# A-Nasiri-M/sap3d_tensorflow

Hardware: AMD Instinct MI355X
Metric: clips/s (16x112x112 fwd+bwd) (higher is better)
Workload: dtype f32

## Files before the change

### sap3d_tensorflow_amd/csrc/elementwise.hip

```cpp
#include "p3d_kernels.h"
#include "det_reduce.h"
#define P3D_SEED(a) ((a).seed_dev ? *(a).seed_dev : (a).seed)

namespace {

__device__ __forceinline__ float4 ld4(const float* p) { return *reinterpret_cast<const float4*>(p); }
__device__ __forceinline__ void st4(float* p, float4 v) { *reinterpret_cast<float4*>(p) = v; }
__device__ __forceinline__ float4 f4(float a) { return make_float4(a, a, a, a); }
__device__ __forceinline__ float4 fma4(float4 a, float4 b, float4 c) {
    return make_float4(fmaf(a.x, b.x, c.x), fmaf(a.y, b.y, c.y), fmaf(a.z, b.z, c.z), fmaf(a.w, b.w, c.w));
}
__device__ __forceinline__ float4 add4(float4 a, float4 b) { return make_float4(a.x + b.x, a.y + b.y, a.z + b.z, a.w + b.w); }
__device__ __forceinline__ float4 sub4(float4 a, float4 b) { return make_float4(a.x - b.x, a.y - b.y, a.z - b.z, a.w - b.w); }
__device__ __forceinline__ float4 mul4(float4 a, float4 b) { return make_float4(a.x * b.x, a.y * b.y, a.z * b.z, a.w * b.w); }
__device__ __forceinline__ float4 relu4(float4 a) { return make_float4(fmaxf(a.x, 0.f), fmaxf(a.y, 0.f), fmaxf(a.z, 0.f), fmaxf(a.w, 0.f)); }
__device__ __forceinline__ float4 gate4(float4 g, float4 pre) {
    return make_float4(pre.x > 0.f ? g.x : 0.f, pre.y > 0.f ? g.y : 0.f, pre.z > 0.f ? g.z : 0.f, pre.w > 0.f ? g.w : 0.f);
}

__device__ __forceinline__ float u01(unsigned long long seed, unsigned long long idx) {
    unsigned long long z = seed + 0x9E3779B97F4A7C15ull * (idx + 1);
    z = (z ^ (z >> 30)) * 0xBF58476D1CE4E5B9ull;
    z = (z ^ (z >> 27)) * 0x94D049BB133111EBull;
    z ^= z >> 31;
    return (float)(z >> 40) * (1.0f / 16777216.0f);
}
__device__ __forceinline__ float4 dropmask4(unsigned long long seed, long long e0, float rate, float scale) {
    return make_float4(u01(seed, e0) >= rate ? scale : 0.f, u01(seed, e0 + 1) >= rate ? scale : 0.f,
                       u01(seed, e0 + 2) >= rate ? scale : 0.f, u01(seed, e0 + 3) >= rate ? scale : 0.f);
}

static_assert(P3D_STAT_REPLICAS == 16, "finalize kernels fold 16 replicas with 4 shuffle steps");
__device__ __forceinline__ double fold16(double v) {
#pragma unroll
    for (int o = 8; o > 0; o >>= 1) v += __shfl_xor(v, o);
    return v;
}
template <int LPC>
__global__ __launch_bounds__(256) void bn_finalize_kernel(BnParams bn, double invM, int use_batch, int update_moving, float eps) {
    P3D_CHAIN_PRIO();
    const int r = threadIdx.x % LPC;
    const int c = blockIdx.x * (256 / LPC) + threadIdx.x / LPC;
    const bool ok = c < bn.C;
    double s1 = 0.0, s2 = 0.0;
    if (use_batch) {
        if (ok) {
            const float2* part = reinterpret_cast<const float2*>(bn.statpart) + c;
#pragma unroll 4
            for (int q = r; q < bn.nparts; q += LPC) {
                const float2 v = part[(size_t)q * bn.C];
                s1 += (double)v.x; s2 += (double)v.y;
            }
        }
#pragma unroll
        for (int o = LPC / 2; o > 0; o >>= 1) { s1 += __shfl_xor(s1, o); s2 += __shfl_xor(s2, o); }
    }
    if (!ok || r) return;
    double mean, var;
    if (use_batch) {
        mean = s1 * invM;
        var = s2 * invM - mean * mean;
        if (var < 0.0) var = 0.0;
        if (update_moving) {
            bn.moving_mean[c] -= (bn.moving_mean[c] - (float)mean) * (1.0f - 0.99f);
            bn.moving_var[c] -= (bn.moving_var[c] - (float)var) * (1.0f - 0.99f);
        }
    } else {
        mean = bn.moving_mean[c];
        var = bn.moving_var[c];
    }
    const double inv = 1.0 / sqrt(var + (double)eps);
    const float sc = (float)((double)bn.gamma[c] * inv);
    bn.scale[c] = sc;
    bn.shift[c] = (float)((double)bn.beta[c] - mean * (double)bn.gamma[c] * inv);
    bn.mean[c] = (float)mean;
    bn.invstd[c] = (float)inv;
}

__global__ __launch_bounds__(256) void bn_stats_kernel(const float* y, int ld, long long M, int C, float* statpart) {
    P3D_CHAIN_PRIO();
    __shared__ float red[256][8];
    const int c4n = C >> 2;
    const int rpi = 256 / c4n;
    const int tid = threadIdx.x;
    const int sub = tid / c4n;
    const int cg = tid - sub * c4n;
    const int c = cg << 2;
    float4 s1 = f4(0.f), s2 = f4(0.f);
    if (sub < rpi)
        for (long long row = (long long)blockIdx.x * rpi + sub; row < M; row += (long long)gridDim.x * rpi) {
            const float4 v = ld4(y + row * ld + c);
            s1 = add4(s1, v);
            s2 = fma4(v, v, s2);
        }
    float* r = red[tid];
    r[0] = s1.x; r[1] = s1.y; r[2] = s1.z; r[3] = s1.w; r[4] = s2.x; r[5] = s2.y; r[6] = s2.z; r[7] = s2.w;
    __syncthreads();
    if (tid < c4n) {
        float t[8];
#pragma unroll
        for (int q = 0; q < 8; ++q) t[q] = 0.f;
        for (int s = 0; s < rpi; ++s)
#pragma unroll
            for (int q = 0; q < 8; ++q) t[q] += red[s * c4n + tid][q];
        float* st = statpart + (size_t)blockIdx.x * 2 * C;
#pragma unroll
        for (int q = 0; q < 4; ++q) { st[2 * (c + q) + 0] = t[q]; st[2 * (c + q) + 1] = t[4 + q]; }
    }
}

template <int MODE>
__global__ __launch_bounds__(256) void bn_apply_kernel(BnApplyArgs a) {
    p3d_warm_kernarg_lines<(int)(sizeof(BnApplyArgs) / 64)>();
    P3D_CHAIN_PRIO();
    const int c4n = a.C >> 2;
    const long long total = a.M * c4n;
    for (long long i = (long long)blockIdx.x * blockDim.x + threadIdx.x; i < total; i += (long long)gridDim.x * blockDim.x) {
        const long long row = i / c4n;
        const int c = (int)(i - row * c4n) << 2;
        float4 v = fma4(ld4(a.scale1 + c), ld4(a.y1 + row * a.ld1 + c), ld4(a.shift1 + c));
        float4 z;
        if (MODE == 0) z = relu4(v);
        else if (MODE == 1) z = relu4(add4(v, ld4(a.y2 + row * a.ld2 + c)));
        else if (MODE == 2) z = relu4(add4(v, fma4(ld4(a.scale2 + c), ld4(a.y2 + row * a.ld2 + c), ld4(a.shift2 + c))));
        else if (MODE == 3) z = add4(relu4(v), relu4(fma4(ld4(a.scale2 + c), ld4(a.y2 + row * a.ld2 + c), ld4(a.shift2 + c))));
        else z = add4(ld4(a.y2 + row * a.ld2 + c), relu4(v));
        if (a.drop_scale > 0.f) z = mul4(z, dropmask4(P3D_SEED(a), row * a.C + c, a.drop_rate, a.drop_scale));
        st4(a.z + row * a.ldz + c, z);
    }
}

__device__ __forceinline__ void bn_fold64(const BnParams& bn, int c0, double invM, int use_batch, int update_moving, float eps, bool publish,
                                          float* sc_lds, float* sh_lds) {
    const int ch = c0 + (threadIdx.x >> 2), r = threadIdx.x & 3;
    double s1 = 0.0, s2 = 0.0;
    if (use_batch) {
        const float2* part = reinterpret_cast<const float2*>(bn.statpart) + ch;
#pragma unroll 8
        for (int q = r; q < bn.nparts; q += 4) {
            const float2 v = part[(size_t)q * bn.C];
            s1 += (double)v.x; s2 += (double)v.y;
        }
        s1 += __shfl_xor(s1, 1); s2 += __shfl_xor(s2, 1);
        s1 += __shfl_xor(s1, 2); s2 += __shfl_xor(s2, 2);
    }
    if (r) return;
    double mean, var;
    if (use_batch) {
        mean = s1 * invM;
        var = s2 * invM - mean * mean;
        if (var < 0.0) var = 0.0;
        if (publish && update_moving) {
            bn.moving_mean[ch] -= (bn.moving_mean[ch] - (float)mean) * (1.0f - 0.99f);
            bn.moving_var[ch] -= (bn.moving_var[ch] - (float)var) * (1.0f - 0.99f);
        }
    } else {
        mean = bn.moving_mean[ch];
        var = bn.moving_var[ch];
    }
    const double inv = 1.0 / sqrt(var + (double)eps);
    const float sc = (float)((double)bn.gamma[ch] * inv);
    const float sh = (float)((double)bn.beta[ch] - mean * (double)bn.gamma[ch] * inv);
    sc_lds[ch - c0] = sc; sh_lds[ch - c0] = sh;
    if (publish) { bn.scale[ch] = sc; bn.shift[ch] = sh; bn.mean[ch] = (float)mean; bn.invstd[ch] = (float)inv; }
}

template <int MODE>
__global__ __launch_bounds__(256) void bn_fold_apply_kernel(BnApplyArgs a, BnParams bn1, BnParams bn2, double invM, int batch1, int batch2,
                                                           int update_moving, float eps, int rows_per_block) {
    p3d_warm_kernarg_lines<(int)((sizeof(BnApplyArgs) + 2 * sizeof(BnParams)) / 64)>();
    P3D_CHAIN_PRIO();
    constexpr bool TWO = (MODE == 2 || MODE == 3);
    __shared__ __attribute__((aligned(16))) float sc1[64], sh1[64], sc2[64], sh2[64];
    const int c0 = blockIdx.y * 64;
    const bool publish = blockIdx.x == 0;
    bn_fold64(bn1, c0, invM, batch1, update_moving, eps, publish, sc1, sh1);
    if (TWO) bn_fold64(bn2, c0, invM, batch2, update_moving, eps, publish, sc2, sh2);
    __syncthreads();
    const int cl = (threadIdx.x & 15) << 2, c = c0 + cl;
    const float4 s1v = ld4(sc1 + cl), h1v = ld4(sh1 + cl);
    float4 s2v = f4(0.f), h2v = f4(0.f);
    if (TWO) { s2v = ld4(sc2 + cl); h2v = ld4(sh2 + cl); }
    const long long r0 = (long long)blockIdx.x * rows_per_block;
    const long long r1 = r0 + rows_per_block < a.M ? r0 + rows_per_block : a.M;
    for (long long row = r0 + (threadIdx.x >> 4); row < r1; row += 16) {
        const float4 v = fma4(s1v, ld4(a.y1 + row * a.ld1 + c), h1v);
        float4 z;
        if (MODE == 0) z = relu4(v);
        else if (MODE == 1) z = relu4(add4(v, ld4(a.y2 + row * a.ld2 + c)));
        else if (MODE == 2) z = relu4(add4(v, fma4(s2v, ld4(a.y2 + row * a.ld2 + c), h2v)));
        else if (MODE == 3) z = add4(relu4(v), relu4(fma4(s2v, ld4(a.y2 + row * a.ld2 + c), h2v)));
        else z = add4(ld4(a.y2 + row * a.ld2 + c), relu4(v));
        st4(a.z + row * a.ldz + c, z);
    }
}

template <int MODE>
__device__ __forceinline__ void bn_bwd_gates(const BnBwdArgs& a, long long row, int c, float4& g1, float4& g2,
                                             float4& y1, float4& y2) {
    float4 dz = ld4(a.dz + row * a.lddz + c);
    if (a.drop_scale > 0.f) dz = mul4(dz, dropmask4(P3D_SEED(a), row * a.C + c, a.drop_rate, a.drop_scale));
    y1 = ld4(a.y1 + row * a.ld1 + c);
    const float4 v1 = fma4(ld4(a.scale1 + c), y1, ld4(a.shift1 + c));
    y2 = f4(0.f);
    if (MODE == 0) { g1 = gate4(dz, v1); g2 = f4(0.f); }
    else if (MODE == 1) { y2 = ld4(a.y2 + row * a.ld2 + c); g1 = gate4(dz, add4(v1, y2)); g2 = g1; }
    else if (MODE == 2) {
        y2 = ld4(a.y2 + row * a.ld2 + c);
        const float4 v2 = fma4(ld4(a.scale2 + c), y2, ld4(a.shift2 + c));
        g1 = gate4(dz, add4(v1, v2)); g2 = g1;
    } else if (MODE == 3) {
        y2 = ld4(a.y2 + row * a.ld2 + c);
        const float4 v2 = fma4(ld4(a.scale2 + c), y2, ld4(a.shift2 + c));
        g1 = gate4(dz, v1); g2 = gate4(dz, v2);
    } else { g1 = gate4(dz, v1); g2 = dz; }
}

template <int MODE>
__global__ __launch_bounds__(256) void bn_bwd_reduce_kernel(BnBwdArgs a) {
    p3d_warm_kernarg_lines<(int)(sizeof(BnBwdArgs) / 64)>();
    P3D_CHAIN_PRIO();
    constexpr bool TWO = (MODE == 2 || MODE == 3);
    __shared__ float red[256][TWO ? 16 : 8];
    const int c4n = a.C >> 2;
    const int rpi = 256 / c4n;
    const int tid = threadIdx.x;
    const int sub = tid / c4n;
    const int cg = tid - sub * c4n;
    const int c = cg << 2;
    const bool active = sub < rpi;
    float4 s1 = f4(0.f), sx1 = f4(0.f), s2 = f4(0.f), sx2 = f4(0.f);
    if (active) {
        const float4 m1 = ld4(a.mean1 + c), i1 = ld4(a.invstd1 + c);
        float4 m2 = f4(0.f), i2 = f4(0.f);
        if (TWO) { m2 = ld4(a.mean2 + c); i2 = ld4(a.invstd2 + c); }
        const long long stride = (long long)gridDim.x * rpi;
        float4 t1 = f4(0.f), tx1 = f4(0.f), t2 = f4(0.f), tx2 = f4(0.f);
        long long row = (long long)blockIdx.x * rpi + sub;
        for (; row + stride < a.M; row += 2 * stride) {
            float4 g1, g2, y1, y2, h1, h2, z1, z2;
            bn_bwd_gates<MODE>(a, row, c, g1, g2, y1, y2);
            bn_bwd_gates<MODE>(a, row + stride, c, h1, h2, z1, z2);
            s1 = add4(s1, g1);
            sx1 = fma4(g1, mul4(sub4(y1, m1), i1), sx1);
            t1 = add4(t1, h1);
            tx1 = fma4(h1, mul4(sub4(z1, m1), i1), tx1);
            if (TWO) {
                s2 = add4(s2, g2);
                sx2 = fma4(g2, mul4(sub4(y2, m2), i2), sx2);
                t2 = add4(t2, h2);
                tx2 = fma4(h2, mul4(sub4(z2, m2), i2), tx2);
            }
        }
        if (row < a.M) {
            float4 g1, g2, y1, y2;
            bn_bwd_gates<MODE>(a, row, c, g1, g2, y1, y2);
            s1 = add4(s1, g1);
            sx1 = fma4(g1, mul4(sub4(y1, m1), i1), sx1);
            if (TWO) {
                s2 = add4(s2, g2);
                sx2 = fma4(g2, mul4(sub4(y2, m2), i2), sx2);
            }
        }
        s1 = add4(s1, t1); sx1 = add4(sx1, tx1);
        if (TWO) { s2 = add4(s2, t2); sx2 = add4(sx2, tx2); }
    }
    float* r = red[tid];
    r[0] = s1.x; r[1] = s1.y; r[2] = s1.z; r[3] = s1.w; r[4] = sx1.x; r[5] = sx1.y; r[6] = sx1.z; r[7] = sx1.w;
    if (TWO) { r[8] = s2.x; r[9] = s2.y; r[10] = s2.z; r[11] = s2.w; r[12] = sx2.x; r[13] = sx2.y; r[14] = sx2.z; r[15] = sx2.w; }
    __syncthreads();
    if (tid < c4n) {
        constexpr int NV = TWO ? 16 : 8;
        float t[NV];
#pragma unroll
        for (int q = 0; q < NV; ++q) t[q] = 0.f;
        for (int s = 0; s < rpi; ++s)
#pragma unroll
            for (int q = 0; q < NV; ++q) t[q] += red[s * c4n + tid][q];
        float* p1 = a.part1 + ((size_t)blockIdx.x * a.C + c) * 2;
#pragma unroll
        for (int q = 0; q < 4; ++q) { p1[2 * q] = t[q]; p1[2 * q + 1] = t[4 + q]; }
        if (TWO) {
            float* p2 = a.part2 + ((size_t)blockIdx.x * a.C + c) * 2;
#pragma unroll
            for (int q = 0; q < 4; ++q) { p2[2 * q] = t[8 + q]; p2[2 * q + 1] = t[12 + q]; }
        }
    }
}

template <int LPC>
__global__ __launch_bounds__(256) void bn_bwd_finalize_kernel(BnBwdArgs a, int two) {
    p3d_warm_kernarg_lines<(int)(sizeof(BnBwdArgs) / 64)>();
    P3D_CHAIN_PRIO();
    const int r = threadIdx.x % LPC;
    const int c = blockIdx.x * (256 / LPC) + threadIdx.x / LPC;
    const bool ok = c < a.C;
    const double invM = 1.0 / (double)a.M;
    double s1 = 0.0, s2 = 0.0, t1 = 0.0, t2 = 0.0;
    if (ok) {
        const float2* p1 = reinterpret_cast<const float2*>(a.part1) + c;
        const float2* p2 = reinterpret_cast<const float2*>(a.part2) + c;
#pragma unroll 4
        for (int q = r; q < a.nparts; q += LPC) {
            const float2 v = p1[(size_t)q * a.C];
            s1 += (double)v.x; s2 += (double)v.y;
            if (two) { const float2 w = p2[(size_t)q * a.C]; t1 += (double)w.x; t2 += (double)w.y; }
        }
    }
#pragma unroll
    for (int o = LPC / 2; o > 0; o >>= 1) {
        s1 += __shfl_xor(s1, o); s2 += __shfl_xor(s2, o);
        if (two) { t1 += __shfl_xor(t1, o); t2 += __shfl_xor(t2, o); }
    }
    if (!ok || r) return;
    a.dbeta1[c] = (float)s1; a.dgamma1[c] = (float)s2;
    a.coef1[2 * c] = (float)(s1 * invM); a.coef1[2 * c + 1] = (float)(s2 * invM);
    if (two) {
        a.dbeta2[c] = (float)t1; a.dgamma2[c] = (float)t2;
        a.coef2[2 * c] = (float)(t1 * invM); a.coef2[2 * c + 1] = (float)(t2 * invM);
    }
}

__global__ __launch_bounds__(256) void bn_grad_finalize_kernel(BnGradFold f) {
    P3D_CHAIN_PRIO();
    const int r = threadIdx.x & 15;
    const int c = blockIdx.x * 16 + (threadIdx.x >> 4);
    const bool ok = c < f.C;
    double sg = 0.0, sgx = 0.0;
    if (ok) {
        const float2* part = reinterpret_cast<const float2*>(f.part) + c;
#pragma unroll 4
        for (int q = r; q < f.nparts; q += 16) {
            const float2 v = part[(size_t)q * f.C];
            sg += (double)v.x; sgx += (double)v.y;
        }
    }
    sg = fold16(sg); sgx = fold16(sgx);
    if (!ok || r) return;
    const float inv = f.invstd[c];
    const float c1 = (float)(sg * f.inv_m), c2 = (float)(sgx * f.inv_m);
    const float k1 = f.gamma[c] * inv;
    const float k2 = -k1 * inv * c2;
    const float k3 = -k1 * c1 - k2 * f.mean[c];
    f.coef[c] = k1; f.coef[f.C + c] = k2; f.coef[2 * f.C + c] = k3;
    f.dgamma[c] = (float)sgx; f.dbeta[c] = (float)sg;
}

__device__ __forceinline__ void ldcoef(const float* coef, int c, float4& c1, float4& c2) {
    const float4 lo = ld4(coef + 2 * c), hi = ld4(coef + 2 * c + 4);
    c1 = make_float4(lo.x, lo.z, hi.x, hi.z);
    c2 = make_float4(lo.y, lo.w, hi.y, hi.w);
}

template <int MODE>
__global__ __launch_bounds__(256) void bn_bwd_apply_kernel(BnBwdArgs a) {
    p3d_warm_kernarg_lines<(int)(sizeof(BnBwdArgs) / 64)>();
    P3D_CHAIN_PRIO();
    constexpr bool TWO = (MODE == 2 || MODE == 3);
    const int c4n = a.C >> 2;
    const long long total = a.M * c4n;
    const long long gtid = (long long)blockIdx.x * blockDim.x + threadIdx.x;
    for (long long i = gtid; i < total; i += (long long)gridDim.x * blockDim.x) {
        const long long row = i / c4n;
        const int c = (int)(i - row * c4n) << 2;
        float4 g1, g2, y1, y2;
        bn_bwd_gates<MODE>(a, row, c, g1, g2, y1, y2);
        {
            const float4 k = mul4(ld4(a.gamma1 + c), ld4(a.invstd1 + c));
            float4 d;
            if (a.batch1) {
                const float4 xh = mul4(sub4(y1, ld4(a.mean1 + c)), ld4(a.invstd1 + c));
                float4 c1, c2;
                ldcoef(a.coef1, c, c1, c2);
                d = mul4(k, sub4(sub4(g1, c1), mul4(xh, c2)));
            } else d = mul4(k, g1);
            float* dst = a.dy1 + row * a.lddy1 + c;
            if (a.acc1) d = add4(d, ld4(dst));
            st4(dst, d);
        }
        if (MODE != 0) {
            float4 d;
            if (TWO) {
                const float4 k = mul4(ld4(a.gamma2 + c), ld4(a.invstd2 + c));
                if (a.batch2) {
                    const float4 xh = mul4(sub4(y2, ld4(a.mean2 + c)), ld4(a.invstd2 + c));
                    float4 c1, c2;
                    ldcoef(a.coef2, c, c1, c2);
                    d = mul4(k, sub4(sub4(g2, c1), mul4(xh, c2)));
                } else d = mul4(k, g2);
            } else d = g2;
            float* dst = a.dy2 + row * a.lddy2 + c;
            if (a.acc2) d = add4(d, ld4(dst));
            st4(dst, d);
        }
    }
}

__global__ __launch_bounds__(256) void maxpool_fwd_kernel(PoolArgs a) {
    p3d_warm_kernarg_lines<(int)(sizeof(PoolArgs) / 64)>();
    P3D_CHAIN_PRIO();
    const int c4n = a.C >> 2;
    const long long total = (long long)a.N * a.Do * a.Ho * a.Wo * c4n;
    for (long long i = (long long)blockIdx.x * blockDim.x + threadIdx.x; i < total; i += (long long)gridDim.x * blockDim.x) {
        long long pos = i / c4n;
        const int c = (int)(i - pos * c4n) << 2;
        const long long opos = pos;
        const int ow = (int)(pos % a.Wo); pos /= a.Wo;
        const int oh = (int)(pos % a.Ho); pos /= a.Ho;
        const int od = (int)(pos % a.Do); const int n = (int)(pos / a.Do);
        float4 best = f4(-INFINITY);
        unsigned bx = 0, by = 0, bz = 0, bw = 0;
        for (int kd = 0; kd < a.kd; ++kd) {
            const int id = od * a.sd - a.pd + kd;
            if ((unsigned)id >= (unsigned)a.Di) continue;
            for (int kh = 0; kh < a.kh; ++kh) {
                const int ih = oh * a.sh - a.ph + kh;
                if ((unsigned)ih >= (unsigned)a.Hi) continue;
                for (int kw = 0; kw < a.kw; ++kw) {
                    const int iw = ow * a.sw - a.pw + kw;
                    if ((unsigned)iw >= (unsigned)a.Wi) continue;
                    const float4 v = ld4(a.x + ((((long long)n * a.Di + id) * a.Hi + ih) * a.Wi + iw) * a.ldx + c);
                    const unsigned t = (unsigned)((kd * a.kh + kh) * a.kw + kw);
                    if (v.x > best.x) { best.x = v.x; bx = t; }
                    if (v.y > best.y) { best.y = v.y; by = t; }
                    if (v.z > best.z) { best.z = v.z; bz = t; }
                    if (v.w > best.w) { best.w = v.w; bw = t; }
                }
            }
        }
        st4(a.y + opos * a.ldy + c, best);
        if (a.idx) a.idx[opos * c4n + (c >> 2)] = bx | (by << 8) | (bz << 16) | (bw << 24);
    }
}

template <int KIND>
__device__ __forceinline__ float loss_term(float z, float p, float t, int through_sigmoid, float& g) {
    if (KIND == 1) {
        g = (through_sigmoid ? p : 1.f / (1.f + expf(-z))) - t;
        return fmaxf(z, 0.f) - z * t + log1pf(expf(-fabsf(z)));
    }
    const float d = p - t;
    const float ad = fabsf(d);
    const bool quad = KIND == 0 && ad < 1.f;
    g = quad ? d : (d > 0.f ? 1.f : (d < 0.f ? -1.f : 0.f));
    if (through_sigmoid) g *= p * (1.f - p);
    return KIND == 2 ? ad : (quad ? 0.5f * d * d : ad - 0.5f);
}

template <int KIND>
__device__ __forceinline__ void loss_body(const float* logits, const float* pred, const float* target, long long n,
                                          double* loss_out, float* dl, int through_sigmoid, int vec4, double* part,
                                          unsigned* counter) {
    __shared__ double wsum[4];
    __shared__ int last_flag;
    double acc = 0.0;
    const bool need_z = KIND == 1, need_p = KIND != 1 || through_sigmoid;
    const long long gtid = (long long)blockIdx.x * blockDim.x + threadIdx.x, gsz = (long long)gridDim.x * blockDim.x;
    if (vec4) {
        const long long n4 = n >> 2;
        for (long long i = gtid; i < n4; i += gsz) {
            const float4 z = need_z ? ld4(logits + 4 * i) : f4(0.f), p = need_p ? ld4(pred + 4 * i) : f4(0.f);
            const float4 t = ld4(target + 4 * i);
            float4 g;
            acc += loss_term<KIND>(z.x, p.x, t.x, through_sigmoid, g.x);
            acc += loss_term<KIND>(z.y, p.y, t.y, through_sigmoid, g.y);
            acc += loss_term<KIND>(z.z, p.z, t.z, through_sigmoid, g.z);
            acc += loss_term<KIND>(z.w, p.w, t.w, through_sigmoid, g.w);
            st4(dl + 4 * i, g);
        }
    } else {
        for (long long i = gtid; i < n; i += gsz)
            acc += loss_term<KIND>(need_z ? logits[i] : 0.f, need_p ? pred[i] : 0.f, target[i], through_sigmoid, dl[i]);
    }
    const double bsum = p3d_block_sum<false>(acc, wsum);
    if (threadIdx.x == 0) p3d_store_wt(part, blockIdx.x, bsum);
    if (!p3d_last_block_wt(counter, gridDim.x, &last_flag)) return;
    double t = 0.0;
    for (unsigned b = threadIdx.x; b < gridDim.x; b += 256) t += part[b];
    t = p3d_block_sum<true>(t, wsum);
    if (threadIdx.x == 0) *loss_out += t;
}
__global__ __launch_bounds__(256) void smooth_l1_kernel(const float* pred, const float* target, long long n,
                                                        double* loss_out, float* dl, int through_sigmoid, int vec4, double* part,
                                                        unsigned* counter) {
    P3D_CHAIN_PRIO();
    loss_body<0>(nullptr, pred, target, n, loss_out, dl, through_sigmoid, vec4, part, counter);
}
__global__ __launch_bounds__(256) void sigmoid_ce_kernel(const float* logits, const float* pred, const float* target, long long n,
                                                         double* loss_out, float* dl, int through_sigmoid, int vec4, double* part,
                                                         unsigned* counter) {
    P3D_CHAIN_PRIO();
    loss_body<1>(logits, pred, target, n, loss_out, dl, through_sigmoid, vec4, part, counter);
}
__global__ __launch_bounds__(256) void l1_loss_kernel(const float* logits, const float* pred, const float* target, long long n,
                                                      double* loss_out, float* dl, int through_sigmoid, int vec4, double* part,
                                                      unsigned* counter) {
// ... 289 lines not shown
        const long long st = gridDim.x;
        for (; row + 7 * st < M; row += 8 * st) {
            float v[8];
#pragma unroll
            for (int u = 0; u < 8; ++u) v[u] = dy[(row + u * st) * ld + c];
#pragma unroll
            for (int u = 0; u < 8; ++u) acc += v[u];
        }
        for (; row < M; row += st) acc += dy[row * ld + c];
        p3d_store_wt(part, (size_t)blockIdx.x * C + c, acc);
    }
    if (!p3d_last_block_wt(counters + blockIdx.y, gridDim.x, &last_flag)) return;
    if (c >= C) return;
    float t = 0.f;
    unsigned b = 0;
    for (; b + 7 < gridDim.x; b += 8) {
        float v[8];
#pragma unroll
        for (int u = 0; u < 8; ++u) v[u] = part[(size_t)(b + u) * C + c];
#pragma unroll
        for (int u = 0; u < 8; ++u) t += v[u];
    }
    for (; b < gridDim.x; ++b) t += part[(size_t)b * C + c];
    out[c] += t;
}

__global__ __launch_bounds__(256) void colsum4_kernel(const float* __restrict__ dy, int ld, long long M, int C, float* out,
                                                      float* part, unsigned* counters) {
    __shared__ float4 red[256];
    __shared__ int last_flag;
    const int L = C >> 2, R = 256 / L;
    const int lane = threadIdx.x % L, rs = threadIdx.x / L;
    const bool live = rs < R;
    float4 acc = make_float4(0.f, 0.f, 0.f, 0.f);
    if (live) {
        const long long stride = (long long)gridDim.x * R;
        long long row = (long long)blockIdx.x * R + rs;
        const float* base = dy + lane * 4;
        for (; row + 7 * stride < M; row += 8 * stride) {
            float4 v[8];
#pragma unroll
            for (int u = 0; u < 8; ++u) v[u] = *reinterpret_cast<const float4*>(base + (row + u * stride) * ld);
#pragma unroll
            for (int u = 0; u < 8; ++u) { acc.x += v[u].x; acc.y += v[u].y; acc.z += v[u].z; acc.w += v[u].w; }
        }
        for (; row < M; row += stride) {
            const float4 v = *reinterpret_cast<const float4*>(base + row * ld);
            acc.x += v.x; acc.y += v.y; acc.z += v.z; acc.w += v.w;
        }
    }
    red[threadIdx.x] = acc;
    __syncthreads();
    if (threadIdx.x < L) {
        float4 t = red[threadIdx.x];
        for (int r = 1; r < R; ++r) { const float4 v = red[r * L + threadIdx.x]; t.x += v.x; t.y += v.y; t.z += v.z; t.w += v.w; }
        p3d_store_wt4(part, (size_t)blockIdx.x * C + threadIdx.x * 4, t);
    }
    if (!p3d_last_block_wt(counters, gridDim.x, &last_flag)) return;
    acc = make_float4(0.f, 0.f, 0.f, 0.f);
    if (live) {
        const float* src = part + lane * 4;
        unsigned b = rs;
        for (; b + 7u * R < gridDim.x; b += 8u * R) {
            float4 v[8];
#pragma unroll
            for (int u = 0; u < 8; ++u) v[u] = *reinterpret_cast<const float4*>(src + (size_t)(b + u * R) * C);
#pragma unroll
            for (int u = 0; u < 8; ++u) { acc.x += v[u].x; acc.y += v[u].y; acc.z += v[u].z; acc.w += v[u].w; }
        }
        for (; b < gridDim.x; b += R) {
            const float4 v = *reinterpret_cast<const float4*>(src + (size_t)b * C);
            acc.x += v.x; acc.y += v.y; acc.z += v.z; acc.w += v.w;
        }
    }
    __syncthreads();
    red[threadIdx.x] = acc;
    __syncthreads();
    if (threadIdx.x < L) {
        float4 t = red[threadIdx.x];
        for (int r = 1; r < R; ++r) { const float4 v = red[r * L + threadIdx.x]; t.x += v.x; t.y += v.y; t.z += v.z; t.w += v.w; }
        float4* o = reinterpret_cast<float4*>(out + threadIdx.x * 4);
        float4 cur = *o;
        cur.x += t.x; cur.y += t.y; cur.z += t.z; cur.w += t.w;
        *o = cur;
    }
}

inline unsigned grid_for(long long total, int per_block = 256, int cap = 4096) {
    long long b = (total + per_block - 1) / per_block;
    if (b < 1) b = 1;
    if (b > cap) b = cap;
    return (unsigned)b;
}

}

hipError_t p3d_bn_finalize(const BnParams& bn, long M, int use_batch, int update_moving, float eps, hipStream_t s) {
    if (use_batch && (!bn.statpart || bn.nparts < 1)) return hipErrorInvalidValue;
    if (use_batch && bn.nparts > 64)
        hipLaunchKernelGGL(bn_finalize_kernel<64>, dim3((bn.C + 3) / 4), dim3(256), 0, s, bn, 1.0 / (double)M, use_batch, update_moving, eps);
    else
        hipLaunchKernelGGL(bn_finalize_kernel<16>, dim3((bn.C + 15) / 16), dim3(256), 0, s, bn, 1.0 / (double)M, use_batch, update_moving, eps);
    return hipGetLastError();
}

int p3d_bn_stats_parts(long M, int C) {
    if ((C & 3) || C > 1024 || C < 4) return 0;
    const int rpi = 256 / (C >> 2);
    long long blocks = (M + (long long)rpi * 8 - 1) / ((long long)rpi * 8);
    if (blocks < 1) blocks = 1;
    if (blocks > 512) blocks = 512;
    return (int)blocks;
}

hipError_t p3d_bn_stats(const float* y, int ld, long M, int C, float* statpart, hipStream_t s) {
    if ((C & 3) || C > 1024 || (ld & 3)) return hipErrorInvalidValue;
    const long long blocks = p3d_bn_stats_parts(M, C);
    hipLaunchKernelGGL(bn_stats_kernel, dim3((unsigned)blocks), dim3(256), 0, s, y, ld, (long long)M, C, statpart);
    return hipGetLastError();
}

hipError_t p3d_bn_apply(const BnApplyArgs& a, hipStream_t s) {
    if ((a.C & 3) || (a.ld1 & 3) || (a.ldz & 3)) return hipErrorInvalidValue;
    const unsigned g = grid_for(a.M * (a.C >> 2));
    switch (a.mode) {
        case 0: hipLaunchKernelGGL(bn_apply_kernel<0>, dim3(g), dim3(256), 0, s, a); break;
        case 1: hipLaunchKernelGGL(bn_apply_kernel<1>, dim3(g), dim3(256), 0, s, a); break;
        case 2: hipLaunchKernelGGL(bn_apply_kernel<2>, dim3(g), dim3(256), 0, s, a); break;
        case 3: hipLaunchKernelGGL(bn_apply_kernel<3>, dim3(g), dim3(256), 0, s, a); break;
        case 4: hipLaunchKernelGGL(bn_apply_kernel<4>, dim3(g), dim3(256), 0, s, a); break;
        default: return hipErrorInvalidValue;
    }
    return hipGetLastError();
}

bool p3d_bn_fold_apply_ok(long M, int C, int nparts1, int nparts2, float drop_scale) {
    static const bool off = p3d_tune_env("P3D_BN_FOLD_APPLY") && atoi(p3d_tune_env("P3D_BN_FOLD_APPLY")) == 0;
    return !off && (C % 64) == 0 && nparts1 <= 128 && nparts2 <= 128 && M >= 1024 && !(drop_scale > 0.f);
}
hipError_t p3d_bn_fold_apply(const BnApplyArgs& a, const BnParams& bn1, const BnParams& bn2, int batch1, int batch2, int update_moving,
                             float eps, hipStream_t s) {
    const bool two = a.mode == 2 || a.mode == 3;
    if ((a.ld1 & 3) || (a.ldz & 3) || !p3d_bn_fold_apply_ok(a.M, a.C, batch1 ? bn1.nparts : 0, two && batch2 ? bn2.nparts : 0, a.drop_scale))
        return hipErrorInvalidValue;
    if ((batch1 && (!bn1.statpart || bn1.nparts < 1)) || (two && batch2 && (!bn2.statpart || bn2.nparts < 1))) return hipErrorInvalidValue;
    const int groups = a.C / 64;
    int chunks = 256 / groups;
    if (chunks < 1) chunks = 1;
    long rows = (a.M + chunks - 1) / chunks;
    rows = (rows + 15) / 16 * 16;
    chunks = (int)((a.M + rows - 1) / rows);
    const dim3 g((unsigned)chunks, (unsigned)groups);
    const double invM = 1.0 / (double)a.M;
#define P3D_FA(M_) case M_: hipLaunchKernelGGL(bn_fold_apply_kernel<M_>, g, dim3(256), 0, s, a, bn1, bn2, invM, batch1, batch2, update_moving, eps, (int)rows); break;
    switch (a.mode) { P3D_FA(0) P3D_FA(1) P3D_FA(2) P3D_FA(3) P3D_FA(4) default: return hipErrorInvalidValue; }
#undef P3D_FA
    return hipGetLastError();
}

int p3d_bn_bwd_parts(long M, int C) {
    if ((C & 3) || C > 1024 || C < 4) return 0;
    const int rpi = 256 / (C >> 2);
    long long blocks = (M + (long long)rpi * 8 - 1) / ((long long)rpi * 8);
    if (blocks < 1) blocks = 1;
    if (blocks > 512) blocks = 512;
    return (int)blocks;
}

hipError_t p3d_bn_bwd_reduce(const BnBwdArgs& a, hipStream_t s) {
    if ((a.C & 3) || a.C > 1024 || !a.part1 || a.nparts != p3d_bn_bwd_parts(a.M, a.C)) return hipErrorInvalidValue;
    const unsigned g = (unsigned)a.nparts;
    switch (a.mode) {
        case 0: hipLaunchKernelGGL(bn_bwd_reduce_kernel<0>, dim3(g), dim3(256), 0, s, a); break;
        case 1: hipLaunchKernelGGL(bn_bwd_reduce_kernel<1>, dim3(g), dim3(256), 0, s, a); break;
        case 2: hipLaunchKernelGGL(bn_bwd_reduce_kernel<2>, dim3(g), dim3(256), 0, s, a); break;
        case 3: hipLaunchKernelGGL(bn_bwd_reduce_kernel<3>, dim3(g), dim3(256), 0, s, a); break;
        case 4: hipLaunchKernelGGL(bn_bwd_reduce_kernel<4>, dim3(g), dim3(256), 0, s, a); break;
        default: return hipErrorInvalidValue;
    }
    return hipGetLastError();
}

hipError_t p3d_bn_bwd_finalize(const BnBwdArgs& a, hipStream_t s) {
    const int two = (a.mode == 2 || a.mode == 3) ? 1 : 0;
    if (a.nparts >= 64) hipLaunchKernelGGL(bn_bwd_finalize_kernel<64>, dim3((a.C + 3) / 4), dim3(256), 0, s, a, two);
    else hipLaunchKernelGGL(bn_bwd_finalize_kernel<16>, dim3((a.C + 15) / 16), dim3(256), 0, s, a, two);
    return hipGetLastError();
}

hipError_t p3d_bn_grad_finalize(const BnGradFold& f, hipStream_t s) {
    if (!f.part || f.nparts <= 0) return hipErrorInvalidValue;
    hipLaunchKernelGGL(bn_grad_finalize_kernel, dim3((f.C + 15) / 16), dim3(256), 0, s, f);
    return hipGetLastError();
}

hipError_t p3d_bn_bwd_apply(const BnBwdArgs& a, hipStream_t s) {
    if (a.C & 3) return hipErrorInvalidValue;
    unsigned g = grid_for(a.M * (a.C >> 2));
    switch (a.mode) {
        case 0: hipLaunchKernelGGL(bn_bwd_apply_kernel<0>, dim3(g), dim3(256), 0, s, a); break;
        case 1: hipLaunchKernelGGL(bn_bwd_apply_kernel<1>, dim3(g), dim3(256), 0, s, a); break;
        case 2: hipLaunchKernelGGL(bn_bwd_apply_kernel<2>, dim3(g), dim3(256), 0, s, a); break;
        case 3: hipLaunchKernelGGL(bn_bwd_apply_kernel<3>, dim3(g), dim3(256), 0, s, a); break;
        case 4: hipLaunchKernelGGL(bn_bwd_apply_kernel<4>, dim3(g), dim3(256), 0, s, a); break;
        default: return hipErrorInvalidValue;
    }
    return hipGetLastError();
}

hipError_t p3d_maxpool_fwd(const PoolArgs& a, hipStream_t s) {
    if (a.C & 3) return hipErrorInvalidValue;
    const long long total = (long long)a.N * a.Do * a.Ho * a.Wo * (a.C >> 2);
    hipLaunchKernelGGL(maxpool_fwd_kernel, dim3(grid_for(total)), dim3(256), 0, s, a);
    return hipGetLastError();
}

__global__ __launch_bounds__(256) void maxpool_bwd_disjoint_kernel(PoolArgs a, int accumulate) {
    p3d_warm_kernarg_lines<(int)(sizeof(PoolArgs) / 64)>();
    P3D_CHAIN_PRIO();
    const int c4n = a.C >> 2;
    const long long total = (long long)a.N * a.Do * a.Ho * a.Wo * c4n;
    for (long long i = (long long)blockIdx.x * blockDim.x + threadIdx.x; i < total; i += (long long)gridDim.x * blockDim.x) {
        long long pos = i / c4n;
        const int c = (int)(i - pos * c4n) << 2;
        const long long opos = pos;
        const int ow = (int)(pos % a.Wo); pos /= a.Wo;
        const int oh = (int)(pos % a.Ho); pos /= a.Ho;
        const int od = (int)(pos % a.Do); const int n = (int)(pos / a.Do);
        const float4 g = ld4(a.dy + opos * a.lddy + c);
        const float4 y = ld4(a.y + opos * a.ldy + c);
        float4 left = g;
        bool done[4] = {false, false, false, false};
        for (int kd = 0; kd < a.kd; ++kd)
            for (int kh = 0; kh < a.kh; ++kh)
                for (int kw = 0; kw < a.kw; ++kw) {
                    const long long ipos = (((long long)n * a.Di + od * a.sd + kd) * a.Hi + oh * a.sh + kh) * a.Wi + ow * a.sw + kw;
                    const float4 v = ld4(a.x + ipos * a.ldx + c);
                    float4 d = f4(0.f);
                    if (!done[0] && v.x == y.x) { d.x = left.x; done[0] = true; }
                    if (!done[1] && v.y == y.y) { d.y = left.y; done[1] = true; }
                    if (!done[2] && v.z == y.z) { d.z = left.z; done[2] = true; }
                    if (!done[3] && v.w == y.w) { d.w = left.w; done[3] = true; }
                    float* dst = a.dx + ipos * a.lddx + c;
                    if (accumulate) d = add4(d, ld4(dst));
                    st4(dst, d);
                }
    }
}

__global__ __launch_bounds__(256) void maxpool_bwd_gather_kernel(PoolArgs a, int accumulate) {
    p3d_warm_kernarg_lines<(int)(sizeof(PoolArgs) / 64)>();
    P3D_CHAIN_PRIO();
    const int c4n = a.C >> 2;
    const long long total = (long long)a.N * a.Di * a.Hi * a.Wi * c4n;
    for (long long i = (long long)blockIdx.x * blockDim.x + threadIdx.x; i < total; i += (long long)gridDim.x * blockDim.x) {
        long long pos = i / c4n;
        const int c = (int)(i - pos * c4n) << 2;
        const long long ipos = pos;
        const int iw = (int)(pos % a.Wi); pos /= a.Wi;
        const int ih = (int)(pos % a.Hi); pos /= a.Hi;
        const int id = (int)(pos % a.Di); const int n = (int)(pos / a.Di);
        const int pdv = id + a.pd, phv = ih + a.ph, pwv = iw + a.pw;
        float4 acc = f4(0.f);
        if (a.kd <= 2 * a.sd && a.kh <= 2 * a.sh && a.kw <= 2 * a.sw) {
            int od2[2], oh2[2], ow2[2];
            bool vd[2], vh[2], vw[2];
#pragma unroll
            for (int q = 0; q < 2; ++q) {
                od2[q] = pdv / a.sd - q; vd[q] = od2[q] >= 0 && od2[q] < a.Do && pdv - od2[q] * a.sd < a.kd;
                oh2[q] = phv / a.sh - q; vh[q] = oh2[q] >= 0 && oh2[q] < a.Ho && phv - oh2[q] * a.sh < a.kh;
                ow2[q] = pwv / a.sw - q; vw[q] = ow2[q] >= 0 && ow2[q] < a.Wo && pwv - ow2[q] * a.sw < a.kw;
            }
            unsigned wd[8]; float4 g8[8]; unsigned t8[8]; bool ok[8];
#pragma unroll
            for (int q = 0; q < 8; ++q) {
                const int qd = q >> 2, qh = (q >> 1) & 1, qw = q & 1;
                ok[q] = vd[qd] && vh[qh] && vw[qw];
                t8[q] = (unsigned)(((pdv - od2[qd] * a.sd) * a.kh + (phv - oh2[qh] * a.sh)) * a.kw + (pwv - ow2[qw] * a.sw));
                const long long opos = ok[q] ? (((long long)n * a.Do + od2[qd]) * a.Ho + oh2[qh]) * a.Wo + ow2[qw] : 0;
                wd[q] = ok[q] ? a.idx[opos * c4n + (c >> 2)] : 0xffffffffu;
                g8[q] = ok[q] ? ld4(a.dy + opos * a.lddy + c) : f4(0.f);
            }
#pragma unroll
            for (int q = 0; q < 8; ++q) {
                if (!ok[q]) continue;
                const unsigned w = wd[q], t = t8[q];
                if ((w & 255u) == t) acc.x += g8[q].x;
                if (((w >> 8) & 255u) == t) acc.y += g8[q].y;
                if (((w >> 16) & 255u) == t) acc.z += g8[q].z;
                if ((w >> 24) == t) acc.w += g8[q].w;
            }
        } else
        for (int od = pdv / a.sd; od >= 0 && pdv - od * a.sd < a.kd; --od) {
            if (od >= a.Do) continue;
            for (int oh = phv / a.sh; oh >= 0 && phv - oh * a.sh < a.kh; --oh) {
                if (oh >= a.Ho) continue;
                for (int ow = pwv / a.sw; ow >= 0 && pwv - ow * a.sw < a.kw; --ow) {
                    if (ow >= a.Wo) continue;
                    const unsigned t = (unsigned)(((pdv - od * a.sd) * a.kh + (phv - oh * a.sh)) * a.kw + (pwv - ow * a.sw));
                    const long long opos = (((long long)n * a.Do + od) * a.Ho + oh) * a.Wo + ow;
                    const unsigned w = a.idx[opos * c4n + (c >> 2)];
                    const float4 g = ld4(a.dy + opos * a.lddy + c);
                    if ((w & 255u) == t) acc.x += g.x;
                    if (((w >> 8) & 255u) == t) acc.y += g.y;
                    if (((w >> 16) & 255u) == t) acc.z += g.z;
                    if ((w >> 24) == t) acc.w += g.w;
                }
            }
        }
        float* dst = a.dx + ipos * a.lddx + c;
        if (accumulate) acc = add4(acc, ld4(dst));
        st4(dst, acc);
    }
}

bool p3d_maxpool_disjoint(const PoolArgs& a) {
    return a.kd == a.sd && a.kh == a.sh && a.kw == a.sw && a.pd == 0 && a.ph == 0 && a.pw == 0 &&
           a.Do * a.sd == a.Di && a.Ho * a.sh == a.Hi && a.Wo * a.sw == a.Wi;
}

hipError_t p3d_maxpool_bwd_disjoint(const PoolArgs& a, int accumulate, hipStream_t s) {
    if ((a.C & 3) || !p3d_maxpool_disjoint(a)) return hipErrorInvalidValue;
    const long long total = (long long)a.N * a.Do * a.Ho * a.Wo * (a.C >> 2);
    hipLaunchKernelGGL(maxpool_bwd_disjoint_kernel, dim3(grid_for(total)), dim3(256), 0, s, a, accumulate);
    return hipGetLastError();
}


static uintptr_t low4(const void* q) { return reinterpret_cast<uintptr_t>(q) & 15; }

LaunchDesc p3d_loss_desc(const LossArgs& a) {
    const double n = (double)a.n;
// ... 245 lines not shown
```

Baseline: 536.2.

## Batch-issue partial-stat and activation loads ahead of reductions in BN kernels

Introduces a PartLoads helper that issues all partial-sum loads up front, with clamped indices, before accumulating them in double. It is used in the BN finalize, backward finalize, grad finalize and fold-apply kernels, and gamma/beta/moving stats are also loaded early. The fold-apply kernel now prefetches several activation rows before finishing the stat fold, so global latency overlaps the fold. The backward reduce adds a single-pass prefetch variant for modes 0 and 4 when each thread covers at most 8 rows. The cost is more registers and more template instantiations, with occupancy risk for the larger prefetch depths.

```diff
diff --git a/sap3d_tensorflow_amd/csrc/elementwise.hip b/sap3d_tensorflow_amd/csrc/elementwise.hip
--- a/sap3d_tensorflow_amd/csrc/elementwise.hip
+++ b/sap3d_tensorflow_amd/csrc/elementwise.hip
@@ -36,43 +36,75 @@
     for (int o = 8; o > 0; o >>= 1) v += __shfl_xor(v, o);
     return v;
 }
+template <int N, int LPC, int TN = N>
+struct PartLoads {
+    float2 v[N];
+    __device__ __forceinline__ void issue(const float2* part, int nparts, int C, int r) {
+#pragma unroll
+        for (int j = 0; j < N; ++j) v[j] = part[(size_t)min(r + j * LPC, nparts - 1) * C];
+    }
+    __device__ __forceinline__ void add(const float2* part, int nparts, int C, int r, double& s1, double& s2) {
+        __builtin_amdgcn_sched_barrier(0);
+#pragma unroll
+        for (int j = 0; j < N; ++j) asm volatile("" : "+v"(v[j].x), "+v"(v[j].y) : : "memory");
+#pragma unroll
+        for (int j = 0; j < N; ++j)
+            if (r + j * LPC < nparts) { s1 += (double)v[j].x; s2 += (double)v[j].y; }
+        for (int q = r + N * LPC; q < nparts; q += TN * LPC) {
+            float2 w[TN];
+#pragma unroll
+            for (int j = 0; j < TN; ++j) w[j] = part[(size_t)min(q + j * LPC, nparts - 1) * C];
+#pragma unroll
+            for (int j = 0; j < TN; ++j)
+                if (q + j * LPC < nparts) { s1 += (double)w[j].x; s2 += (double)w[j].y; }
+        }
+    }
+};
+
 template <int LPC>
 __global__ __launch_bounds__(256) void bn_finalize_kernel(BnParams bn, double invM, int use_batch, int update_moving, float eps) {
+    p3d_warm_kernarg_lines<(int)((sizeof(BnParams) + sizeof(double) + 2 * sizeof(int) + sizeof(float) + 63) / 64)>();
     P3D_CHAIN_PRIO();
+    constexpr int N = LPC == 64 ? 8 : 4;
+    constexpr int TN = LPC == 64 ? 16 : 4;
     const int r = threadIdx.x % LPC;
     const int c = blockIdx.x * (256 / LPC) + threadIdx.x / LPC;
     const bool ok = c < bn.C;
+    const bool last = ok && r == 0;
+    float g = 0.f, b = 0.f, mm = 0.f, mv = 0.f;
+    if (last) {
+        g = bn.gamma[c]; b = bn.beta[c];
+        if (!use_batch || update_moving) { mm = bn.moving_mean[c]; mv = bn.moving_var[c]; }
+    }
     double s1 = 0.0, s2 = 0.0;
     if (use_batch) {
         if (ok) {
             const float2* part = reinterpret_cast<const float2*>(bn.statpart) + c;
-#pragma unroll 4
-            for (int q = r; q < bn.nparts; q += LPC) {
-                const float2 v = part[(size_t)q * bn.C];
-                s1 += (double)v.x; s2 += (double)v.y;
-            }
+            PartLoads<N, LPC, TN> p;
+            p.issue(part, bn.nparts, bn.C, r);
+            p.add(part, bn.nparts, bn.C, r, s1, s2);
         }
 #pragma unroll
         for (int o = LPC / 2; o > 0; o >>= 1) { s1 += __shfl_xor(s1, o); s2 += __shfl_xor(s2, o); }
     }
-    if (!ok || r) return;
+    if (!last) return;
     double mean, var;
     if (use_batch) {
         mean = s1 * invM;
         var = s2 * invM - mean * mean;
         if (var < 0.0) var = 0.0;
         if (update_moving) {
-            bn.moving_mean[c] -= (bn.moving_mean[c] - (float)mean) * (1.0f - 0.99f);
-            bn.moving_var[c] -= (bn.moving_var[c] - (float)var) * (1.0f - 0.99f);
+            bn.moving_mean[c] = mm - (mm - (float)mean) * (1.0f - 0.99f);
+            bn.moving_var[c] = mv - (mv - (float)var) * (1.0f - 0.99f);
         }
     } else {
-        mean = bn.moving_mean[c];
-        var = bn.moving_var[c];
+        mean = mm;
+        var = mv;
     }
     const double inv = 1.0 / sqrt(var + (double)eps);
-    const float sc = (float)((double)bn.gamma[c] * inv);
+    const float sc = (float)((double)g * inv);
     bn.scale[c] = sc;
-    bn.shift[c] = (float)((double)bn.beta[c] - mean * (double)bn.gamma[c] * inv);
+    bn.shift[c] = (float)((double)b - mean * (double)g * inv);
     bn.mean[c] = (float)mean;
     bn.invstd[c] = (float)inv;
 }
@@ -130,17 +162,25 @@
     }
 }
 
-__device__ __forceinline__ void bn_fold64(const BnParams& bn, int c0, double invM, int use_batch, int update_moving, float eps, bool publish,
-                                          float* sc_lds, float* sh_lds) {
+struct BnFold64 {
+    PartLoads<32, 4> p;
+    float g, b, mm, mv;
+};
+__device__ __forceinline__ void bn_fold64_issue(BnFold64& f, const BnParams& bn, int c0, int use_batch, int update_moving, bool publish) {
+    const int ch = c0 + (threadIdx.x >> 2), r = threadIdx.x & 3;
+    f.g = f.b = f.mm = f.mv = 0.f;
+    if (use_batch) f.p.issue(reinterpret_cast<const float2*>(bn.statpart) + ch, bn.nparts, bn.C, r);
+    if (r == 0) {
+        f.g = bn.gamma[ch]; f.b = bn.beta[ch];
+        if (!use_batch || (publish && update_moving)) { f.mm = bn.moving_mean[ch]; f.mv = bn.moving_var[ch]; }
+    }
+}
+__device__ __forceinline__ void bn_fold64_finish(BnFold64& f, const BnParams& bn, int c0, double invM, int use_batch, int update_moving,
+                                                 float eps, bool publish, float* sc_lds, float* sh_lds) {
     const int ch = c0 + (threadIdx.x >> 2), r = threadIdx.x & 3;
     double s1 = 0.0, s2 = 0.0;
     if (use_batch) {
-        const float2* part = reinterpret_cast<const float2*>(bn.statpart) + ch;
-#pragma unroll 8
-        for (int q = r; q < bn.nparts; q += 4) {
-            const float2 v = part[(size_t)q * bn.C];
-            s1 += (double)v.x; s2 += (double)v.y;
-        }
+        f.p.add(reinterpret_cast<const float2*>(bn.statpart) + ch, bn.nparts, bn.C, r, s1, s2);
         s1 += __shfl_xor(s1, 1); s2 += __shfl_xor(s2, 1);
         s1 += __shfl_xor(s1, 2); s2 += __shfl_xor(s2, 2);
     }
@@ -151,47 +191,70 @@
         var = s2 * invM - mean * mean;
         if (var < 0.0) var = 0.0;
         if (publish && update_moving) {
-            bn.moving_mean[ch] -= (bn.moving_mean[ch] - (float)mean) * (1.0f - 0.99f);
-            bn.moving_var[ch] -= (bn.moving_var[ch] - (float)var) * (1.0f - 0.99f);
+            bn.moving_mean[ch] = f.mm - (f.mm - (float)mean) * (1.0f - 0.99f);
+            bn.moving_var[ch] = f.mv - (f.mv - (float)var) * (1.0f - 0.99f);
         }
     } else {
-        mean = bn.moving_mean[ch];
-        var = bn.moving_var[ch];
+        mean = f.mm;
+        var = f.mv;
     }
     const double inv = 1.0 / sqrt(var + (double)eps);
-    const float sc = (float)((double)bn.gamma[ch] * inv);
-    const float sh = (float)((double)bn.beta[ch] - mean * (double)bn.gamma[ch] * inv);
+    const float sc = (float)((double)f.g * inv);
+    const float sh = (float)((double)f.b - mean * (double)f.g * inv);
     sc_lds[ch - c0] = sc; sh_lds[ch - c0] = sh;
     if (publish) { bn.scale[ch] = sc; bn.shift[ch] = sh; bn.mean[ch] = (float)mean; bn.invstd[ch] = (float)inv; }
 }
 
 template <int MODE>
+__device__ __forceinline__ float4 bn_fold_apply_row(float4 y1, float4 y2, float4 s1v, float4 h1v, float4 s2v, float4 h2v) {
+    const float4 v = fma4(s1v, y1, h1v);
+    if (MODE == 0) return relu4(v);
+    else if (MODE == 1) return relu4(add4(v, y2));
+    else if (MODE == 2) return relu4(add4(v, fma4(s2v, y2, h2v)));
+    else if (MODE == 3) return add4(relu4(v), relu4(fma4(s2v, y2, h2v)));
+    else return add4(y2, relu4(v));
+}
+
+template <int MODE, int PF>
 __global__ __launch_bounds__(256) void bn_fold_apply_kernel(BnApplyArgs a, BnParams bn1, BnParams bn2, double invM, int batch1, int batch2,
                                                            int update_moving, float eps, int rows_per_block) {
     p3d_warm_kernarg_lines<(int)((sizeof(BnApplyArgs) + 2 * sizeof(BnParams)) / 64)>();
     P3D_CHAIN_PRIO();
     constexpr bool TWO = (MODE == 2 || MODE == 3);
+    constexpr int NPF = PF > 0 ? PF : 1;
     __shared__ __attribute__((aligned(16))) float sc1[64], sh1[64], sc2[64], sh2[64];
+    if (PF > 0) batch1 = batch2 = 1;
     const int c0 = blockIdx.y * 64;
     const bool publish = blockIdx.x == 0;
-    bn_fold64(bn1, c0, invM, batch1, update_moving, eps, publish, sc1, sh1);
-    if (TWO) bn_fold64(bn2, c0, invM, batch2, update_moving, eps, publish, sc2, sh2);
+    const int cl = (threadIdx.x & 15) << 2, c = c0 + cl;
+    const long long r0 = (long long)blockIdx.x * rows_per_block;
+    const long long r1 = r0 + rows_per_block < a.M ? r0 + rows_per_block : a.M;
+    const long long row0 = r0 + (threadIdx.x >> 4);
+    BnFold64 f1, f2;
+    bn_fold64_issue(f1, bn1, c0, batch1, update_moving, publish);
+    if (TWO) bn_fold64_issue(f2, bn2, c0, batch2, update_moving, publish);
+    float4 y1v[NPF], y2v[NPF];
+#pragma unroll
+    for (int j = 0; j < PF; ++j) {
+        const long long row = row0 + 16 * j < a.M ? row0 + 16 * j : a.M - 1;
+        y1v[j] = ld4(a.y1 + row * a.ld1 + c);
+        y2v[j] = MODE != 0 ? ld4(a.y2 + row * a.ld2 + c) : f4(0.f);
+    }
+    bn_fold64_finish(f1, bn1, c0, invM, batch1, update_moving, eps, publish, sc1, sh1);
+    if (TWO) bn_fold64_finish(f2, bn2, c0, invM, batch2, update_moving, eps, publish, sc2, sh2);
     __syncthreads();
-    const int cl = (threadIdx.x & 15) << 2, c = c0 + cl;
     const float4 s1v = ld4(sc1 + cl), h1v = ld4(sh1 + cl);
     float4 s2v = f4(0.f), h2v = f4(0.f);
     if (TWO) { s2v = ld4(sc2 + cl); h2v = ld4(sh2 + cl); }
-    const long long r0 = (long long)blockIdx.x * rows_per_block;
-    const long long r1 = r0 + rows_per_block < a.M ? r0 + rows_per_block : a.M;
-    for (long long row = r0 + (threadIdx.x >> 4); row < r1; row += 16) {
-        const float4 v = fma4(s1v, ld4(a.y1 + row * a.ld1 + c), h1v);
-        float4 z;
-        if (MODE == 0) z = relu4(v);
-        else if (MODE == 1) z = relu4(add4(v, ld4(a.y2 + row * a.ld2 + c)));
-        else if (MODE == 2) z = relu4(add4(v, fma4(s2v, ld4(a.y2 + row * a.ld2 + c), h2v)));
-        else if (MODE == 3) z = add4(relu4(v), relu4(fma4(s2v, ld4(a.y2 + row * a.ld2 + c), h2v)));
-        else z = add4(ld4(a.y2 + row * a.ld2 + c), relu4(v));
-        st4(a.z + row * a.ldz + c, z);
+#pragma unroll
+    for (int j = 0; j < PF; ++j) {
+        const long long row = row0 + 16 * j;
+        if (row < r1) st4(a.z + row * a.ldz + c, bn_fold_apply_row<MODE>(y1v[j], y2v[j], s1v, h1v, s2v, h2v));
+    }
+    for (long long row = row0 + 16 * PF; row < r1; row += 16) {
+        float4 y2 = f4(0.f);
+        if (MODE != 0) y2 = ld4(a.y2 + row * a.ld2 + c);
+        st4(a.z + row * a.ldz + c, bn_fold_apply_row<MODE>(ld4(a.y1 + row * a.ld1 + c), y2, s1v, h1v, s2v, h2v));
     }
 }
 
@@ -216,7 +279,7 @@
     } else { g1 = gate4(dz, v1); g2 = dz; }
 }
 
-template <int MODE>
+template <int MODE, bool PRE>
 __global__ __launch_bounds__(256) void bn_bwd_reduce_kernel(BnBwdArgs a) {
     p3d_warm_kernarg_lines<(int)(sizeof(BnBwdArgs) / 64)>();
     P3D_CHAIN_PRIO();
@@ -237,7 +300,31 @@
         const long long stride = (long long)gridDim.x * rpi;
         float4 t1 = f4(0.f), tx1 = f4(0.f), t2 = f4(0.f), tx2 = f4(0.f);
         long long row = (long long)blockIdx.x * rpi + sub;
-        for (; row + stride < a.M; row += 2 * stride) {
+        if constexpr (PRE) {
+            static_assert(MODE == 0 || MODE == 4, "the sums of modes 1-3 read y2 as well: the loop");
+            const float4 sc1 = ld4(a.scale1 + c), sh1 = ld4(a.shift1 + c);
+            const unsigned long long seed = a.drop_scale > 0.f ? P3D_SEED(a) : 0ull;
+            float4 dzv[8], y1v[8];
+#pragma unroll
+            for (int k = 0; k < 8; ++k) {
+                const long long rk = row + k * stride < a.M ? row + k * stride : a.M - 1;
+                dzv[k] = ld4(a.dz + rk * a.lddz + c);
+                y1v[k] = ld4(a.y1 + rk * a.ld1 + c);
+            }
+#pragma unroll
+            for (int k = 0; k < 8; ++k) {
+                const long long rk = row + k * stride;
+                if (rk < a.M) {
+                    float4 dz = dzv[k];
+                    if (a.drop_scale > 0.f) dz = mul4(dz, dropmask4(seed, rk * a.C + c, a.drop_rate, a.drop_scale));
+                    const float4 g1 = gate4(dz, fma4(sc1, y1v[k], sh1));
+                    const float4 x1 = mul4(sub4(y1v[k], m1), i1);
+                    if (k & 1) { t1 = add4(t1, g1); tx1 = fma4(g1, x1, tx1); }
+                    else { s1 = add4(s1, g1); sx1 = fma4(g1, x1, sx1); }
+                }
+            }
+        }
+        for (; !PRE && row + stride < a.M; row += 2 * stride) {
             float4 g1, g2, y1, y2, h1, h2, z1, z2;
             bn_bwd_gates<MODE>(a, row, c, g1, g2, y1, y2);
             bn_bwd_gates<MODE>(a, row + stride, c, h1, h2, z1, z2);
@@ -252,7 +339,7 @@
                 tx2 = fma4(h2, mul4(sub4(z2, m2), i2), tx2);
             }
         }
-        if (row < a.M) {
+        if (!PRE && row < a.M) {
             float4 g1, g2, y1, y2;
             bn_bwd_gates<MODE>(a, row, c, g1, g2, y1, y2);
             s1 = add4(s1, g1);
@@ -296,16 +383,16 @@
     const int c = blockIdx.x * (256 / LPC) + threadIdx.x / LPC;
     const bool ok = c < a.C;
     const double invM = 1.0 / (double)a.M;
+    constexpr int N = LPC == 64 ? 8 : 4;
     double s1 = 0.0, s2 = 0.0, t1 = 0.0, t2 = 0.0;
     if (ok) {
         const float2* p1 = reinterpret_cast<const float2*>(a.part1) + c;
         const float2* p2 = reinterpret_cast<const float2*>(a.part2) + c;
-#pragma unroll 4
-        for (int q = r; q < a.nparts; q += LPC) {
-            const float2 v = p1[(size_t)q * a.C];
-            s1 += (double)v.x; s2 += (double)v.y;
-            if (two) { const float2 w = p2[(size_t)q * a.C]; t1 += (double)w.x; t2 += (double)w.y; }
-        }
+        PartLoads<N, LPC> v, w;
+        v.issue(p1, a.nparts, a.C, r);
+        if (two) w.issue(p2, a.nparts, a.C, r);
+        v.add(p1, a.nparts, a.C, r, s1, s2);
+        if (two) w.add(p2, a.nparts, a.C, r, t1, t2);
     }
 #pragma unroll
     for (int o = LPC / 2; o > 0; o >>= 1) {
@@ -327,21 +414,20 @@
     const int c = blockIdx.x * 16 + (threadIdx.x >> 4);
     const bool ok = c < f.C;
     double sg = 0.0, sgx = 0.0;
+    float inv = 0.f, gamma = 0.f, mean = 0.f;
+    if (ok && r == 0) { inv = f.invstd[c]; gamma = f.gamma[c]; mean = f.mean[c]; }
     if (ok) {
         const float2* part = reinterpret_cast<const float2*>(f.part) + c;
-#pragma unroll 4
-        for (int q = r; q < f.nparts; q += 16) {
-            const float2 v = part[(size_t)q * f.C];
-            sg += (double)v.x; sgx += (double)v.y;
-        }
+        PartLoads<8, 16> v;
+        v.issue(part, f.nparts, f.C, r);
+        v.add(part, f.nparts, f.C, r, sg, sgx);
     }
     sg = fold16(sg); sgx = fold16(sgx);
     if (!ok || r) return;
-    const float inv = f.invstd[c];
     const float c1 = (float)(sg * f.inv_m), c2 = (float)(sgx * f.inv_m);
-    const float k1 = f.gamma[c] * inv;
+    const float k1 = gamma * inv;
     const float k2 = -k1 * inv * c2;
-    const float k3 = -k1 * c1 - k2 * f.mean[c];
+    const float k3 = -k1 * c1 - k2 * mean;
     f.coef[c] = k1; f.coef[f.C + c] = k2; f.coef[2 * f.C + c] = k3;
     f.dgamma[c] = (float)sgx; f.dbeta[c] = (float)sg;
 }
@@ -937,8 +1023,13 @@
     chunks = (int)((a.M + rows - 1) / rows);
     const dim3 g((unsigned)chunks, (unsigned)groups);
     const double invM = 1.0 / (double)a.M;
-#define P3D_FA(M_) case M_: hipLaunchKernelGGL(bn_fold_apply_kernel<M_>, g, dim3(256), 0, s, a, bn1, bn2, invM, batch1, batch2, update_moving, eps, (int)rows); break;
+    const long rpt = rows / 16;
+    const int pf = !(batch1 && (!two || batch2)) ? 0 : rpt <= 4 ? 4 : (rpt <= 8 || two) ? 8 : 16;
+#define P3D_FA_PF(M_, PF_) hipLaunchKernelGGL((bn_fold_apply_kernel<M_, PF_>), g, dim3(256), 0, s, a, bn1, bn2, invM, batch1, batch2, update_moving, eps, (int)rows)
+#define P3D_FA(M_) case M_: if (pf == 0) P3D_FA_PF(M_, 0); else if (pf == 4) P3D_FA_PF(M_, 4); else if (pf == 8) P3D_FA_PF(M_, 8); \
+                            else if constexpr (M_ != 2 && M_ != 3) P3D_FA_PF(M_, 16); break;
     switch (a.mode) { P3D_FA(0) P3D_FA(1) P3D_FA(2) P3D_FA(3) P3D_FA(4) default: return hipErrorInvalidValue; }
+#undef P3D_FA_PF
 #undef P3D_FA
     return hipGetLastError();
 }
@@ -953,16 +1044,15 @@
 }
 
 hipError_t p3d_bn_bwd_reduce(const BnBwdArgs& a, hipStream_t s) {
-    if ((a.C & 3) || a.C > 1024 || !a.part1 || a.nparts != p3d_bn_bwd_parts(a.M, a.C)) return hipErrorInvalidValue;
+    if ((a.C & 3) || a.C < 4 || a.C > 1024 || !a.part1 || a.nparts != p3d_bn_bwd_parts(a.M, a.C)) return hipErrorInvalidValue;
     const unsigned g = (unsigned)a.nparts;
-    switch (a.mode) {
-        case 0: hipLaunchKernelGGL(bn_bwd_reduce_kernel<0>, dim3(g), dim3(256), 0, s, a); break;
-        case 1: hipLaunchKernelGGL(bn_bwd_reduce_kernel<1>, dim3(g), dim3(256), 0, s, a); break;
-        case 2: hipLaunchKernelGGL(bn_bwd_reduce_kernel<2>, dim3(g), dim3(256), 0, s, a); break;
-        case 3: hipLaunchKernelGGL(bn_bwd_reduce_kernel<3>, dim3(g), dim3(256), 0, s, a); break;
-        case 4: hipLaunchKernelGGL(bn_bwd_reduce_kernel<4>, dim3(g), dim3(256), 0, s, a); break;
-        default: return hipErrorInvalidValue;
-    }
+    const bool pre = (a.mode == 0 || a.mode == 4) && a.nparts <= 256 && a.M >= 1 && a.M <= 8ll * a.nparts * (256 / (a.C >> 2));
+#define P3D_BR(M_) case M_: hipLaunchKernelGGL((bn_bwd_reduce_kernel<M_, false>), dim3(g), dim3(256), 0, s, a); break;
+#define P3D_BR_PRE(M_) case M_: if (pre) hipLaunchKernelGGL((bn_bwd_reduce_kernel<M_, true>), dim3(g), dim3(256), 0, s, a); \
+                                else hipLaunchKernelGGL((bn_bwd_reduce_kernel<M_, false>), dim3(g), dim3(256), 0, s, a); break;
+    switch (a.mode) { P3D_BR_PRE(0) P3D_BR(1) P3D_BR(2) P3D_BR(3) P3D_BR_PRE(4) default: return hipErrorInvalidValue; }
+#undef P3D_BR_PRE
+#undef P3D_BR
     return hipGetLastError();
 }
 
```

New measurement: 537.9, median of 2. No clear change (+0.3%).
